# ChampiB/CBO_with_OOP

Measured on AMD Instinct MI355X. Metric: candidate-intervention acquisitions/sec (16k grid, d=3), higher is better.
Workload: dtype f64

## Files before the change

### cbo_with_oop_amd/csrc/cbo_api.hip

```cpp
#include <algorithm>
#include <atomic>
#include <cmath>
#include <cstdio>
#include <cstdlib>
#include <chrono>
#include <cstring>
#include <mutex>
#include <string>
#include <map>
#include <utility>
#include <vector>

#include "cbo_internal.h"
#include "hyper_prior.h"
#include "lml_outputs.h"
#include "schedule_tuner.h"

using namespace cbo;

static thread_local std::string g_err;
static std::atomic<uint64_t> g_fit_stamp{0};

static int fail(int code, const std::string &msg)
{
// ... 347 lines not shown
                if (c->bulk_stream) { hipStreamDestroy(c->bulk_stream); c->bulk_stream = nullptr; }
            }
        }
        if (!masked) {
            e = hipStreamCreateWithPriority(&c->sweep_stream, hipStreamNonBlocking, (prio_low + prio_high) / 2);
            if (e == hipSuccess) e = hipStreamCreateWithPriority(&c->bulk_stream, hipStreamNonBlocking, prio_low);
        }
    }
    if (e == hipSuccess) e = hipEventCreateWithFlags(&c->ev_join, hipEventDisableTiming | hipEventDisableSystemFence);
    if (e == hipSuccess) e = hipEventCreateWithFlags(&c->ev_join2, hipEventDisableTiming | hipEventDisableSystemFence);
    if (e == hipSuccess) e = hipEventCreateWithFlags(&c->ev_fork, hipEventDisableTiming | hipEventDisableSystemFence);
    if (e == hipSuccess) e = hipMalloc(&c->part_val, 2048 * sizeof(double));
    if (e == hipSuccess) e = hipMalloc(&c->part_idx, 2048 * sizeof(int64_t));
    if (e == hipSuccess) e = hipMalloc(&c->best_val, sizeof(double));
    if (e == hipSuccess) e = hipMalloc(&c->best_idx, sizeof(int64_t));
    if (e == hipSuccess) e = hipHostMalloc(&c->h_best_val, sizeof(double));
    if (e == hipSuccess) e = hipHostMalloc(&c->h_best_idx, sizeof(int64_t));
    if (e == hipSuccess) e = hipHostMalloc(&c->h_info, sizeof(int));
    if (e == hipSuccess) e = hipHostMalloc(&c->stage, kStageBytes);
    if (e == hipSuccess) e = hipEventCreateWithFlags(&c->stage_done, hipEventDisableTiming);
    if (e != hipSuccess) {
        destroy_ctx(c);
        return fail(CBO_ERR_HIP, std::string("cbo_init: ") + hipGetErrorString(e));
    }
    const char *ws = std::getenv("CBO_HIP_WORKSPACE_MB");
    if (ws) c->max_ws_bytes = (size_t)std::atoll(ws) << 20;
    c->n_cu = prop.multiProcessorCount;
    const char *sm = std::getenv("CBO_HIP_SWEEP");
    if (sm) c->sweep_mode = std::atoi(sm);
    const char *lr = std::getenv("CBO_HIP_LOO_ROUTE");
    if (lr) c->loo_route = std::atoi(lr);
    const char *hs = std::getenv("CBO_HIP_HYPER_SCHEDULE");
    if (hs) c->hyper_schedule = std::atoi(hs);
    const char *sc = std::getenv("CBO_HIP_SWEEP_CACHE");
    if (sc && std::atoi(sc) == 0) c->sweep_cache = false;
    const char *ss = std::getenv("CBO_HIP_SMALL_SETS");
    if (ss && std::atoi(ss) == 0) c->small_sets = false;
    const char *om = std::getenv("CBO_HIP_OVERLAP");
    if (om) c->overlap_mode = std::atoi(om);
    const char *tf = std::getenv("CBO_HIP_PIPE_TAIL");
    if (tf) c->pipe_tail_frac = std::atof(tf);
    const char *pg = std::getenv("CBO_HIP_PIPE_GROUP");
    if (pg) c->pipe_group = std::min(std::max(std::atoi(pg), 0), 4);
    const char *pl = std::getenv("CBO_HIP_PIPE_LEAD");
    if (pl) c->pipe_lead = std::atoi(pl);
    const char *pf = std::getenv("CBO_HIP_PANEL_FORM");
    if (pf && (std::atoi(pf) == 2 || std::atoi(pf) == 5)) c->chol.panel_form = std::atoi(pf);
    const char *sl = std::getenv("CBO_HIP_FUSED_SPIN_LIMIT");
    if (sl) c->chol.spin_limit = std::atoi(sl);
    const char *bg = std::getenv("CBO_HIP_BULK_GROUP");
    if (bg) c->chol.bulk_group = std::atoi(bg);
    const char *g4 = std::getenv("CBO_HIP_BULK_GROUP4_ROWS");
    if (g4) c->chol.group4_rows = std::atoi(g4);
    const char *vf = std::getenv("CBO_HIP_VEC_SOLVE_FORM");
    if (vf) c->vec_solve_form = std::atoi(vf);
    {
        static std::once_flag once;
        std::call_once(once, [] { std::atexit(shutdown_all_at_exit); });
        std::lock_guard<std::mutex> lock(g_live_mutex);
        g_live.push_back(c);
    }
    *out = c;
    return CBO_OK;
}

namespace cbo {
hipStream_t ctx_stream(cbo_ctx *c) { return c->stream; }
int ctx_device(cbo_ctx *c) { return c->device; }
}

extern "C" void cbo_shutdown(cbo_ctx *c)
{
    if (!c) return;
    {
        std::lock_guard<std::mutex> lock(g_live_mutex);
        auto it = std::find(g_live.begin(), g_live.end(), c);
        if (it == g_live.end()) return;
        g_live.erase(it);
    }
    destroy_ctx(c);
}

static void destroy_ctx(cbo_ctx *c)
{
    hipSetDevice(c->device);
    if (c->scratch_k) { cbo_cands_destroy(c->scratch_k); c->scratch_k = nullptr; }
    if (c->stream) hipStreamSynchronize(c->stream);
    for (auto &p : c->pending) { hipEventDestroy(p.a); hipEventDestroy(p.b); }
    for (auto e : c->pool) hipEventDestroy(e);
    hipFree(c->part_val); hipFree(c->part_idx); hipFree(c->best_val); hipFree(c->best_idx);
    hipHostFree(c->h_best_val); hipHostFree(c->h_best_idx); hipHostFree(c->h_info); hipHostFree(c->stage);
    if (c->stage_done) hipEventDestroy(c->stage_done);
    for (auto e : c->chol_events) hipEventDestroy(e);
    for (auto e : c->pipe_events) hipEventDestroy(e);
    if (c->region_a) hipEventDestroy(c->region_a);
    if (c->region_b) hipEventDestroy(c->region_b);
    if (c->ev_join) hipEventDestroy(c->ev_join);
    if (c->ev_join2) hipEventDestroy(c->ev_join2);
    if (c->ev_fork) hipEventDestroy(c->ev_fork);
    if (c->sweep_stream) hipStreamDestroy(c->sweep_stream);
    if (c->bulk_stream) hipStreamDestroy(c->bulk_stream);
    if (c->side_stream) hipStreamDestroy(c->side_stream);
    if (c->stream) hipStreamDestroy(c->stream);
    delete c;
}

// ... 665 lines not shown
    const int64_t max_cols = (int64_t)(c->max_ws_bytes / (elem * (size_t)n_pad)) / kStrip * kStrip;
    if (cols > max_cols) cols = max_cols < kStrip ? kStrip : max_cols;
    const int64_t ld = cols + (int64_t)(128 / elem);
    int rc = grow(c, c->V, (elem * (size_t)n_pad * (size_t)ld + sizeof(double) - 1) / sizeof(double));
    if (rc == CBO_OK) rc = grow_vectors(c, m_pad);
    if (rc != CBO_OK) return rc;
    *chunk_cols = cols;
    *ldv = ld;
    return CBO_OK;
}

static int prepare_cands(cbo_gp *g, cbo_cands *k)
{
    cbo_ctx *c = g->ctx;
    if (k->prepared_for == g && k->prepared_ls == g->ls) return CBO_OK;
    launch_prep_points(c->stream, k->raw, k->m, k->d, g->h.ard ? g->ls_dev : nullptr, k->has_prior ? k->pv : nullptr,
                       k->P.xs, k->m_pad, k->P.sq, k->has_prior ? k->P.sv : nullptr);
    HIP_TRY(hipGetLastError());
    k->prepared_for = g;
    k->prepared_ls = g->ls;
    return CBO_OK;
}

static void pipe_mark(void *user, hipStream_t st, int begin, double flops)
{
    cbo_ctx *c = static_cast<cbo_ctx *>(user);
    if (!c->profiling) return;
    EventPair &cur = c->pipe_cur;
    if (begin) {
        cur.a = get_event(c);
        cur.b = get_event(c);
        cur.phase = PH_TRSM;
        hipEventRecord(cur.a, st);
        c->timers.n_trsm_launches += 1;
        c->timers.trsm_flops += flops;
    } else {
        hipEventRecord(cur.b, st);
        c->pending.push_back(cur);
    }
}

static SweepPipe make_pipe(cbo_gp *g, double *V, int64_t ldv, int64_t cols, double *q, double *mu)
{
    cbo_ctx *c = g->ctx;
    SweepPipe pipe{};
    pipe.stream = c->sweep_stream;
    pipe.bulk = c->bulk_stream;
    pipe.V = V; pipe.ldv = ldv; pipe.m_pad = cols;
    pipe.zvec = g->z; pipe.q = q; pipe.mu = mu;
    pipe.events = &c->pipe_events;
    pipe.mark = pipe_mark; pipe.user = c;
    pipe.tail_begin = (int)g->n_pad;
    pipe.group = 0;
    return pipe;
}

static bool prefer_right_looking(const cbo_ctx *c, int64_t n_pad, int64_t cols)
{
    if (c->sweep_mode == 0) return false;
    if (c->sweep_mode == 1) return true;
    if (n_pad < 1024) return false;
    const int64_t strips = cols / kStrip;
    const int64_t rounds = (strips + c->n_cu - 1) / c->n_cu;
    return rounds * c->n_cu * 5 >= strips * 6;
}


static int enqueue_right_looking(cbo_gp *g, double *V, int64_t ldv, int64_t cols, double *q, double *mu,
                                 bool lower_tri = false)
{
    cbo_ctx *c = g->ctx;
    SweepPipe pipe = make_pipe(g, V, ldv, cols, q, mu);
    pipe.lower_tri = lower_tri;
    HIP_TRY(hipMemsetAsync(q, 0, sizeof(double) * cols, c->stream));
    HIP_TRY(hipMemsetAsync(mu, 0, sizeof(double) * cols, c->stream));
    int p = 0;
    for (int r0 = 0; r0 < (int)g->n_pad; r0 += 256, ++p)
        sweep_pipe_pair(pipe, c->stream, g->A, g->lda, g->invDt, g->n_pad, p, r0,
                        (r0 + 256 <= (int)g->n_pad) ? 256 : 128);
    HIP_TRY(hipEventRecord(c->ev_join, c->sweep_stream));
    HIP_TRY(hipStreamWaitEvent(c->stream, c->ev_join, 0));
    HIP_TRY(hipEventRecord(c->ev_join2, c->bulk_stream));
    HIP_TRY(hipStreamWaitEvent(c->stream, c->ev_join2, 0));
    return CBO_OK;
}

static int own_solution_buffer(cbo_gp *g, cbo_cands *k, double **V, int64_t *ldv)
{
    cbo_ctx *c = g->ctx;
    if (!k->V || k->v_rows_cap != g->n_pad || k->v_ld != k->m_pad + kLdExtra) {
        HIP_TRY(hipStreamSynchronize(c->stream));
        hipFree(k->V); hipFree(k->partial);
        k->V = nullptr; k->partial = nullptr; k->v_stamp = 0;
        k->v_ld = k->m_pad + kLdExtra;
        HIP_TRY(hipMalloc(&k->V, sizeof(double) * (size_t)g->n_pad * (size_t)k->v_ld));
        HIP_TRY(hipMalloc(&k->partial, sizeof(double) * 64 * (size_t)k->m_pad));
        k->v_rows_cap = g->n_pad;
    }
    *V = k->V;
    *ldv = k->v_ld;
    return CBO_OK;
}

static int enqueue_posterior_f32(cbo_gp *g, cbo_cands *k)
{
    cbo_ctx *c = g->ctx;
// ... 3042 lines not shown
    for (int j = 0, q = 0; j < ns + nm; ++j) {
        const cbo_mle_run &r = runs[taken[(size_t)j]];
        const size_t P = (size_t)r.n_params;
        for (int s = 0; s < r.n_starts; ++s, ++q) {
            if (c->mle_status[q] == kNoStatus) return fail(CBO_ERR_HIP, "MLE kernel: no status for a run it was given");
            r.status_out[s] = c->mle_status[q];
            r.rounds_out[s] = c->mle_rounds[q];
            if (r.status_out[s] == CBO_MLE_NOT_PD) continue;
            const double *fin = c->mle_final.p + (size_t)q * kFinal;
            std::memcpy(r.theta_out + (size_t)s * P, fin, sizeof(double) * P);
            r.lml_out[s] = fin[CBO_HMC_MAX_PARAMS];
            std::memcpy(r.grad_out + (size_t)s * P, fin + CBO_HMC_MAX_PARAMS + 1, sizeof(double) * P);
        }
    }
    return CBO_OK;
}

extern "C" int cbo_gp_mle_sets(int n_models, cbo_gp *const *gps, const cbo_mle_run *runs, int *model_status_out)
{
    return cbo_gp_mle_sets_rows(n_models, gps, runs, kPadN, model_status_out);
}

static int general_lml_gradients(cbo_gp *g, double *lml_out, double *dvariance_out, double *dlengthscale_out,
                                 double *dnoise_out)
{
    cbo_ctx *c = g->ctx;
    if (!g->fitted) {
        if (g->n_pad != kPadN) return fail(CBO_ERR_NOT_FITTED, "gp is not fitted");
        const int frc = cbo_gp_fit(g, nullptr, nullptr);
        if (frc != CBO_OK) return frc;
    }
    int rc = ensure_alpha(g);
    if (rc != CBO_OK) return rc;
    const int64_t n_pad = g->n_pad;
    int64_t chunk = 0, ldv = 0;
    rc = ensure_workspaces(c, n_pad, n_pad, &chunk, &ldv);
    if (rc != CBO_OK) return rc;
    if (chunk < n_pad) return fail(CBO_ERR_UNSUPPORTED, "likelihood gradients need an n_pad x n_pad workspace (raise CBO_HIP_WORKSPACE_MB)");
    const int64_t ldw = n_pad + kLdExtra;
    const size_t w_bytes = sizeof(double) * (size_t)n_pad * (size_t)ldw;
    rc = grow(c, c->W, (size_t)n_pad * (size_t)ldw);
    if (rc == CBO_OK) rc = grow(c, c->gpart, (size_t)lml_grad_tiles(n_pad) * (size_t)(1 + g->d));
    if (rc != CBO_OK) return rc;
    launch_set_identity(c->stream, c->V, ldv, n_pad);
    if (prefer_right_looking(c, n_pad, n_pad)) {
        rc = enqueue_right_looking(g, c->V, ldv, n_pad, c->q, c->mu, true);
        if (rc != CBO_OK) return rc;
    } else {
        launch_trsm_strips(c->stream, g->A, g->lda, g->invDt, c->V, ldv, n_pad, n_pad, g->z, c->q, c->mu);
    }
    HIP_TRY(hipMemsetAsync(c->W, 0, w_bytes, c->stream));
    for (int k0 = 0; k0 < (int)n_pad; k0 += 256) {
        const int klen = (k0 + 256 <= (int)n_pad) ? 256 : 128;
        launch_gemm_update(c->stream, c->V, ldv, c->V, ldv, c->W, ldw, k0, klen, 0, k0 + klen, k0 + klen, true);
    }
    launch_lml_grad(c->stream, g->X, g->h, g->alpha, c->W, ldw, n_pad, c->gpart, c->part_val);
    launch_lml_terms(c->stream, g->A, g->lda, n_pad, g->z, c->part_val + 16);
    HIP_TRY(hipGetLastError());
    launch_dot2(c->stream, g->alpha, g->alpha, g->n, c->part_val + 20);
    launch_sum(c->stream, c->q, g->n, c->part_val + 22);
    HIP_TRY(hipGetLastError());
    double hs[24];
    HIP_TRY(hipMemcpyAsync(hs, c->part_val, sizeof(hs), hipMemcpyDeviceToHost, c->stream));
    HIP_TRY(hipStreamSynchronize(c->stream));
    lml_outputs(g, hs, hs[16], hs[17], hs[20], hs[22], lml_out, dvariance_out, dlengthscale_out, dnoise_out);
    return CBO_OK;
}

static int general_loo(cbo_gp *g, double *mean_out, double *var_out, double *lpd_out, double *sum_out)
{
    cbo_ctx *c = g->ctx;
    int rc = ensure_alpha(g);
    if (rc != CBO_OK) return rc;
    const int64_t n_pad = g->n_pad;
    int64_t chunk = 0, ldv = 0;
    rc = ensure_workspaces(c, n_pad, n_pad, &chunk, &ldv);
    if (rc != CBO_OK) return rc;
    const int nb = loo_finish_blocks(g->n);
    rc = grow(c, c->gpart, (size_t)nb + 1);
    if (rc != CBO_OK) return rc;
    if (c->loo_route != 1 && c->loo_route != 2 && chunk >= n_pad && prefer_right_looking(c, n_pad, n_pad)) {
        launch_set_identity(c->stream, c->V, ldv, n_pad);
        rc = enqueue_right_looking(g, c->V, ldv, n_pad, c->q, c->mu, true);
        if (rc != CBO_OK) return rc;
    } else {
        for (int64_t c0 = 0; c0 < n_pad; c0 += chunk) {
            const int64_t cols = (n_pad - c0 < chunk) ? (n_pad - c0) : chunk;
            const int64_t r0 = c->loo_route == 2 ? 0 : c0 / 256 * 256;
            const int64_t rows = n_pad - r0;
            PhaseScope ps(c, PH_TRSM);
            launch_loo_identity_chunk(c->stream, c->V, ldv, rows, cols, c0 - r0);
            launch_trsm_strips(c->stream, g->A + r0 * g->lda + r0, g->lda, g->invDt + (r0 / 16) * 256, c->V, ldv, rows,
                               cols, g->z + r0, c->q + c0, c->mu + c0);
            if (c->profiling) {
                c->timers.n_trsm_launches += 1;
                c->timers.trsm_flops += (double)rows * (double)rows * (double)cols;
            }
        }
    }
    double *partial = c->gpart, *sum_dev = c->gpart + nb;
    launch_loo_finish(c->stream, c->q, g->alpha, g->y, g->n, mean_out ? c->mean.p : nullptr, var_out ? c->var.p : nullptr,
                      lpd_out ? c->acq.p : nullptr, partial, sum_dev);
    HIP_TRY(hipGetLastError());
    const size_t bytes = sizeof(double) * (size_t)g->n;
    if (mean_out) HIP_TRY(hipMemcpyAsync(mean_out, c->mean, bytes, hipMemcpyDeviceToHost, c->stream));
    if (var_out) HIP_TRY(hipMemcpyAsync(var_out, c->var, bytes, hipMemcpyDeviceToHost, c->stream));
    if (lpd_out) HIP_TRY(hipMemcpyAsync(lpd_out, c->acq, bytes, hipMemcpyDeviceToHost, c->stream));
// ... 452 lines not shown
```

### cbo_with_oop_amd/csrc/cbo_internal.h

```cpp
#pragma once

#include <hip/hip_runtime.h>
#include <cstddef>
#include <cstdint>
#include <string>
#include <vector>

#include "cbo_hip.h"

namespace cbo {

typedef double d4 __attribute__((ext_vector_type(4)));
typedef double d2 __attribute__((ext_vector_type(2)));

#if defined(__HIP_DEVICE_COMPILE__) || defined(__HIPCC__)
typedef __attribute__((address_space(3))) void *lds_ptr_t;
__device__ __forceinline__ void glds16(const double *gsrc, unsigned lds_dst)
{
    unsigned keep;
    asm volatile("s_mov_b32 %0, m0\n\ts_mov_b32 m0, %2\n\ts_nop 0\n\tglobal_load_lds_dwordx4 %1, off\n\ts_mov_b32 m0, %0"
                 : "=&s"(keep)
                 : "v"(gsrc), "s"(lds_dst)
                 : "memory");
}
// ... 58 lines not shown
    int n_k;
    const double *xs1, *sq1, *sv1, *xs2, *sq2, *sv2; int64_t ldx;
    int64_t m1, m2;
    double *C; int64_t ldc;
    double variance, inv_l2, noise;
    int zero_diag, tiles;
};
void launch_cov_tiles(hipStream_t s, int d, bool sym, CovArgs a);
struct SampArgs {
    const double *U; int64_t ldu;
    const double *Z; int64_t ldz;
    const double *mean;
    int64_t m, s;
    double *F; int64_t ldf;
    int tiles_i, tiles_j;
};
void launch_samples_tiles(hipStream_t st, SampArgs a);
void launch_normals_transpose(hipStream_t st, const double *normals, int64_t m, int64_t s, double *Z, int64_t m_pad,
                              int64_t ldz);
void launch_factor_padding(hipStream_t st, double *A, int64_t lda, int64_t m, int64_t m_pad);
constexpr int kJointTile = 128;
struct IvrArgs {
    const double *Vc, *Vi; int64_t ldv, c_cols, i_cols;
    int n_k;
    const double *xs1, *sq1, *sv1, *xs2, *sq2, *sv2; int64_t ldx;
    int64_t m, p;
    double *part; int64_t ldp; int64_t tile0;
    double variance, inv_l2;
};
void launch_ivr_tiles(hipStream_t s, int d, IvrArgs a);
void launch_ivr_finish(hipStream_t s, const double *part, int64_t ldp, int tiles, const double *var, int64_t m, double p,
                       double cost, double *ivr, double *part_val, int64_t *part_idx, int n_blocks);
int ivr_finish_blocks_for(int64_t m);
constexpr int kPadN32 = 256;
void launch_factor_to_f32(hipStream_t s, const double *A, int64_t lda, int64_t n_pad, const double *invDt, float *Uf,
                          int64_t ldu, float *invF, int64_t n32);
void launch_kstar_f32(hipStream_t s, const PointSet &X, const PointSet &C, int64_t c_begin, int64_t m_pad,
                      const KernelHyper &h, float *V, int64_t ldv, int64_t n32, const double *alpha, double *mu_part,
                      double *mu);
void launch_trsm_strips_f32(hipStream_t s, const float *U, int64_t ldu, const float *invDt, float *V, int64_t ldv,
                            int64_t n32, int64_t m_pad, double *q);
int run_mfma_f32_selftest(hipStream_t s, double *max_err);

struct SweepPipe {
    hipStream_t stream;
    hipStream_t bulk;
    double *V;
    int64_t ldv, m_pad;
    double *zvec;
    double *q, *mu;
    bool lower_tri;
    int group;
    int lead = 0;
    int tail_begin;
    std::vector<hipEvent_t> *events;
    void (*mark)(void *user, hipStream_t st, int begin, double flops);
    void *user;
};
constexpr int kCholFlagSlots = 1024;
constexpr int kCholFusedTimeout = -2147483647 - 1;
constexpr int kFusedSpinLimit = 1 << 22;
struct CholOptions {
    int panel_form = 4;
    int spin_limit = kFusedSpinLimit;
    int bulk_group = 4;
    int group4_rows = 10240;
};
void launch_cholesky(hipStream_t s, hipStream_t side, std::vector<hipEvent_t> &events, double *A, int64_t lda,
                     int64_t n_pad, double *invDt, int *info_dev, const CholOptions &opt, const SweepPipe *pipe = nullptr,
                     bool info_zeroed = false);
inline int cholesky_info_ints(int64_t n_pad)
{
    const int np = (int)(n_pad / 128);
    return 2 * np <= kCholFlagSlots ? 1 + 2 * np : 1;
}
void sweep_pipe_pair(const SweepPipe &pipe, hipStream_t chain, const double *A, int64_t lda, const double *invDt,
                     int64_t n_pad, int p, int r0, int klen);
void sweep_pipe_tail(const SweepPipe &pipe, hipStream_t chain, const double *A, int64_t lda, const double *invDt,
                     int64_t n_pad, int pairs_done);
void launch_backsolve(hipStream_t s, const double *A, int64_t lda, int64_t n_pad, const double *invDt, double *alpha);
void launch_forward_vec(hipStream_t s, const double *A, int64_t lda, int64_t n_pad, const double *invDt, double *w,
                        double *out);
void launch_gather_column(hipStream_t s, const double *V, int64_t ldv, int64_t n_pad, double *dst);
bool launch_backsolve_chain(hipStream_t s, const double *A, int64_t lda, int64_t n_pad, const double *invDt,
                            const double *src, int64_t src_stride, double *work, double *out, int *info, int spin_limit,
                            int form);
bool launch_forward_chain(hipStream_t s, const double *A, int64_t lda, int64_t n_pad, const double *invDt, const double *w,
                          double *out, int *info, int spin_limit, int form);
void launch_backsolve_vec(hipStream_t s, const double *A, int64_t lda, int64_t n_pad, const double *invDt,
                          const double *src, int64_t src_stride, double *work, double *out);
void launch_pred_gradients(hipStream_t s, const PointSet &X, int64_t n_pad, const PointSet &C, int64_t c_begin,
                           int64_t cols, int64_t m, const KernelHyper &h, const double *inv_ls_dev, const double *alpha,
                           const double *W, int64_t ldw, double *dmean, double *dvar);
void launch_reversed_factor(hipStream_t s, const double *A, int64_t lda, int64_t n_pad, const double *invDt, double *T,
                            int64_t ldt, double *invT);
void launch_reverse_rows(hipStream_t s, const double *V, int64_t ldv, int64_t n_pad, int64_t cols, double *W, int64_t ldw);
void launch_dot2(hipStream_t s, const double *a, const double *b, int64_t n, double *out2);
void launch_sum(hipStream_t s, const double *a, int64_t n, double *out);
void launch_expand_interventions(hipStream_t s, const double *observed, int64_t n_obs, int d, const double *values, int n_iv,
                                 const int *iv_index, int64_t m, double *raw);

void launch_trsm_strips(hipStream_t s, const double *U, int64_t ldu, const double *invDt, double *V, int64_t ldv,
                        int64_t n, int64_t m_pad, const double *z, double *q, double *mu, bool accumulate = false,
                        bool half_lds = false);
void launch_gemm_update(hipStream_t s, const double *U, int64_t ldu, const double *V, int64_t ldv, double *C,
                        int64_t ldc, int k0, int klen, int i0_begin, int i0_end, int64_t m_pad, bool upper_only,
                        const int *skip_if = nullptr);

struct cbo_small_set {
    const double *xs, *sq, *sv, *pm, *y;
    const double *cxs, *csq, *csv, *cpm, *cpv;
    int64_t ld, cld, m, index_offset;
    int n, d, zero_diag, task;
    double variance, lengthscale, noise_var, diag_add, y_best, ei_jitter, cost;
    int ard, pad_;
    const double *stage, *stage_ls;
    double *raw, *pv;
};
struct cbo_small_result {
    double best_val;
    int64_t best_idx;
    int info;
    int seq;
};
size_t small_sets_scratch_doubles(int n_sets, int blocks_per_set);
constexpr int kSmallLmlTerms = 1 + CBO_MAX_DIM + 4;
struct cbo_small_lml_result {
    double terms[kSmallLmlTerms];
    int info, seq;
};
size_t small_lml_scratch_doubles();
void launch_small_lml(hipStream_t s, const cbo_small_set &st, double *scratch, int *info, cbo_small_lml_result *out, int seq);
size_t mid_lml_scratch_doubles();
void launch_small_lml_batch(hipStream_t s, const cbo_small_set *sets, int n_models, double *scratch, int64_t stride,
                            int *info, cbo_small_lml_result *out, int seq);
struct cbo_small_loo_result {
    double sum;
    double mean[128], var[128], lpd[128];
    int info, seq;
};
size_t small_loo_scratch_doubles();
void launch_small_loo_batch(hipStream_t s, const cbo_small_set *sets, int n_models, double *scratch, int *info,
                            cbo_small_loo_result *out, int seq);
void launch_loo_identity_chunk(hipStream_t s, double *V, int64_t ldv, int64_t rows, int64_t cols, int64_t shift);
int loo_finish_blocks(int64_t n);
void launch_loo_finish(hipStream_t s, const double *c, const double *alpha, const double *y, int64_t n, double *mean_out,
                       double *var_out, double *lpd_out, double *partial, double *sum_out);
constexpr int kSmallTwoPhaseFromBlocks = 12;
constexpr int kEiKind = 0;
constexpr int kMesKind = 5;
constexpr int kPredictKind = 6;
constexpr int kLogEiKind = 7;
constexpr int kEiPointKind = 8;
constexpr int kLogEiPointKind = 9;
struct cbo_small_aux {
    int64_t off, count;
};
struct SmallAux {
    const cbo_small_aux *per_set = nullptr;
    const double *data = nullptr;
// ... 283 lines not shown
```

### cbo_with_oop_amd/csrc/kernels_chol.hip

```cpp
#include <hip/hip_ext.h>
#include <climits>
#include <atomic>
#include <cstring>
#include <vector>

#include "cbo_mid_lml_device.h"

namespace cbo {

__global__ __launch_bounds__(256) void potrf_diag128_v2_kernel(double *A, int64_t lda, int r0, int rcol,
                                                               double *__restrict__ invDt, int *info,
                                                               double *__restrict__ zvec)
{
    extern __shared__ __align__(16) unsigned char smem_raw[];
    Diag2Shared &sh = *reinterpret_cast<Diag2Shared *>(smem_raw);
    if (__builtin_nontemporal_load(info) != 0) return;
    const int tid = threadIdx.x;
    const int lane = tid & 63;
    const int wave = __builtin_amdgcn_readfirstlane(tid >> 6);
    {
        const unsigned s0 = lds_byte_address(&sh.S[0][0]);
        const double *g = A + (int64_t)(r0 + wave * 32) * lda + r0 + lane * 2;
#pragma unroll 8
        for (int p = 0; p < 32; ++p) {
// ... 469 lines not shown
static void launch_syrk_rows(hipStream_t s, double *A, int64_t lda, int r0, int n1, int n2, int rcol, const int *skip_if,
                             int rows = 128, hipEvent_t done = nullptr)
{
    const int c0 = r0 + n1;
    const int nt = n2 / 64;
    if (nt <= 0) { if (done) hipEventRecord(done, s); return; }
    if (rows > n2) rows = n2;
    hipExtLaunchKernelGGL(syrk_rows_kernel, dim3(nt + 1, rows / 32), dim3(256), 0, s, nullptr, done, 0, A, lda, r0, n1, c0,
                          nt, rcol, skip_if);
}

static void launch_syrk(hipStream_t s, double *A, int64_t lda, int r0, int n1, int n2, int rcol, int ti_begin,
                        int ti_end, const int *skip_if)
{
    const int c0 = r0 + n1;
    const int nt = n2 / 64;
    if (ti_end > nt) ti_end = nt;
    if (ti_end <= ti_begin) return;
    hipLaunchKernelGGL(syrk_kernel<64>, dim3(nt + 1, ti_end - ti_begin), dim3(256), 0, s, A, lda, r0, n1, c0, nt, rcol,
                       ti_begin, skip_if);
}

static hipEvent_t event_slot(std::vector<hipEvent_t> &ev, size_t i)
{
    while (ev.size() <= i) {
        hipEvent_t e;
        hipEventCreateWithFlags(&e, hipEventDisableTiming | hipEventDisableSystemFence);
        ev.push_back(e);
    }
    return ev[i];
}

void sweep_pipe_pair(const SweepPipe &pipe, hipStream_t chain, const double *A, int64_t lda, const double *invDt,
                     int64_t n_pad, int p, int r0, int klen)
{
    auto pipe_event = [&](int kind, int pp) {
        return event_slot(*pipe.events, (size_t)(3 * pp + kind));
    };
    const int64_t cols = (pipe.lower_tri && r0 + klen < pipe.m_pad) ? (int64_t)(r0 + klen) : pipe.m_pad;
    const double m = (double)cols;
    hipEventRecord(pipe_event(0, p), chain);
    hipStreamWaitEvent(pipe.stream, pipe_event(0, p), 0);
    if (pipe.mark) pipe.mark(pipe.user, pipe.stream, 1, (double)klen * (double)klen * m);
    launch_trsm_strips(pipe.stream, A + (int64_t)r0 * lda + r0, lda, invDt + (int64_t)(r0 / 16) * 256,
                       pipe.V + (int64_t)r0 * pipe.ldv, pipe.ldv, klen, cols, pipe.zvec + r0, pipe.q, pipe.mu, true, true);
    if (pipe.mark) pipe.mark(pipe.user, pipe.stream, 0, 0.0);
    hipEventRecord(pipe_event(1, p), pipe.stream);
    const int below = r0 + klen;
    if (below >= (int)n_pad) return;
    const int first_end = (below + 256 < (int)n_pad) ? below + 256 : (int)n_pad;
    auto update = [&](hipStream_t st, int k0, int kl, int i0, int i1) {
        if (i0 >= i1) return;
        if (pipe.mark) pipe.mark(pipe.user, st, 1, 2.0 * (double)kl * (double)(i1 - i0) * m);
        launch_gemm_update(st, A, lda, pipe.V, pipe.ldv, pipe.V, pipe.ldv, k0, kl, i0, i1, cols, false);
        if (pipe.mark) pipe.mark(pipe.user, st, 0, 0.0);
    };
    const int G = pipe.group, lead = pipe.lead;
    const int full_pairs = ((pipe.tail_begin < (int)n_pad) ? pipe.tail_begin : (int)n_pad) / 256;
    const bool grouped = G >= 2 && !pipe.lower_tri && klen == 256 && p >= lead && ((p - lead) / G + 1) * G + lead <= full_pairs;
    if (grouped) {
        const int j = (p - lead) / G, i = (p - lead) % G;
        const int g0 = 256 * (lead + G * j);
        const int next_end = (g0 + 512 * G < (int)n_pad) ? g0 + 512 * G : (int)n_pad;
        if (i == 0 && j == 0 && lead > 0) hipStreamWaitEvent(pipe.stream, pipe_event(2, lead - 1), 0);
        update(pipe.stream, r0, 256, below, first_end);
        if (i == 0 && j >= 1) hipStreamWaitEvent(pipe.stream, pipe_event(2, lead + G * (j - 1)), 0);
        update(pipe.stream, r0, 256, r0 + 512, next_end);
        if (i < G - 1) return;
        hipStreamWaitEvent(pipe.bulk, pipe_event(1, p), 0);
        const int a1 = (g0 + 768 * G < (int)n_pad) ? g0 + 768 * G : (int)n_pad;
        update(pipe.bulk, g0, 256 * G, next_end, a1);
        hipEventRecord(pipe_event(2, lead + G * j), pipe.bulk);
        update(pipe.bulk, g0, 256 * G, a1, (int)n_pad);
        hipEventRecord(pipe_event(2, p), pipe.bulk);
        return;
    }
    if (p > 0) hipStreamWaitEvent(pipe.stream, pipe_event(2, p - 1), 0);
    update(pipe.stream, r0, klen, below, first_end);
    hipStreamWaitEvent(pipe.bulk, pipe_event(1, p), 0);
    update(pipe.bulk, r0, klen, first_end, (int)n_pad);
    hipEventRecord(pipe_event(2, p), pipe.bulk);
}

void sweep_pipe_tail(const SweepPipe &pipe, hipStream_t chain, const double *A, int64_t lda, const double *invDt,
                     int64_t n_pad, int pairs_done)
{
    std::vector<hipEvent_t> &ev = *pipe.events;
    const hipEvent_t last = event_slot(ev, (size_t)(3 * pairs_done));
    if (pairs_done > 0) {
        hipEventRecord(last, pipe.stream);
        hipStreamWaitEvent(chain, last, 0);
        hipStreamWaitEvent(chain, ev[(size_t)(3 * (pairs_done - 1) + 2)], 0);
    }
    const int t0 = pipe.tail_begin;
    const double rows = (double)((int)n_pad - t0);
    if (pipe.mark) pipe.mark(pipe.user, chain, 1, rows * rows * (double)pipe.m_pad);
    launch_trsm_strips(chain, A + (int64_t)t0 * lda + t0, lda, invDt + (int64_t)(t0 / 16) * 256,
                       pipe.V + (int64_t)t0 * pipe.ldv, pipe.ldv, (int64_t)n_pad - t0, pipe.m_pad, pipe.zvec + t0, pipe.q,
                       pipe.mu, true, false);
    if (pipe.mark) pipe.mark(pipe.user, chain, 0, 0.0);
}

__global__ void zero_ints_kernel(int *p, int n)
{
    for (int i = threadIdx.x; i < n; i += blockDim.x) p[i] = 0;
}

void launch_cholesky(hipStream_t s, hipStream_t side, std::vector<hipEvent_t> &events, double *A, int64_t lda,
                     int64_t n_pad, double *invDt, int *info_dev, const CholOptions &opt, const SweepPipe *pipe,
                     bool info_zeroed)
{
    hipFuncSetAttribute(reinterpret_cast<const void *>(potrf_diag128_v2_kernel), hipFuncAttributeMaxDynamicSharedMemorySize,
                        (int)sizeof(Diag2Shared));
    hipFuncSetAttribute(reinterpret_cast<const void *>(panel_trsm_kernel), hipFuncAttributeMaxDynamicSharedMemorySize,
                        (int)sizeof(PanelShared));
    hipFuncSetAttribute(reinterpret_cast<const void *>(potrf_panel_fused_kernel), hipFuncAttributeMaxDynamicSharedMemorySize,
                        (int)sizeof(Diag2Shared));
    constexpr int syrk_gemm_rows = 6144;
    auto launch_diag = [&](int rr) {
        hipLaunchKernelGGL(potrf_diag128_v2_kernel, dim3(1), dim3(256), sizeof(Diag2Shared), s, A, lda, rr, (int)n_pad,
                           invDt, info_dev, pipe ? pipe->zvec : nullptr);
    };
    const int np = (int)(n_pad / 128);
    const bool fused = opt.panel_form != 2 && 2 * np <= kCholFlagSlots;
    const bool split = opt.panel_form == 5;
    if (!info_zeroed) hipLaunchKernelGGL(zero_ints_kernel, dim3(1), dim3(256), 0, s, info_dev, fused ? 1 + 2 * np : 1);
    int *flags = info_dev + 1;
    const int rcol = (int)n_pad;
    event_slot(events, (size_t)(2 * np + 1));
    hipEventRecord(events[2 * np], s);
    hipStreamWaitEvent(side, events[2 * np], 0);
    double *zvec = pipe ? pipe->zvec : nullptr;
    const bool lean_panel = !pipe;
    int pair = 0;
    auto sweep_rows = [&](int r0, int klen) {
        if (pipe && r0 < pipe->tail_begin) sweep_pipe_pair(*pipe, s, A, lda, invDt, n_pad, pair++, r0, klen);
    };
    int pending = -1;
    int group_left = 0;
    int group_pairs = 0, group_g0 = 0, group_first_k = 0;
    int pending_big_a = -1;
    for (int k = 0; k < np; k += 2) {
        const int r0 = 128 * k;
        const int n2 = (int)n_pad - r0 - 128;
        const int n3_pair = (int)n_pad - r0 - 256;
        if (group_left == 0 && opt.bulk_group >= 2 && (fused || lean_panel)) {
            int G = 0;
            if (opt.bulk_group >= 4 && n3_pair - 1024 >= opt.group4_rows && n3_pair - 1024 >= syrk_gemm_rows &&
                n3_pair - 1024 >= 1024)
                G = 4;
            else if (n3_pair - 512 >= syrk_gemm_rows && n3_pair - 512 >= 512) G = 2;
            if (G != 0) { group_pairs = G; group_left = G; group_g0 = r0; group_first_k = k; }
        }
        const bool grouped = group_left > 0;
        const bool first_of_group = grouped && group_left == group_pairs;
        const bool last_of_group = grouped && group_left == 1;
        const bool split_now = split || grouped;
        auto factor_panel = [&](int r, int cols, hipEvent_t done) {
            if (fused && cols > 0) {
                launch_panel_fused(s, A, lda, r, rcol, invDt, info_dev, zvec, cols, flags + 2 * (r / 128), opt.spin_limit,
                                   done, split_now);
                return;
            }
            launch_diag(r);
            if (cols <= 0) return;
            if (lean_panel) launch_panel_trsm(s, A, lda, r, r + 128, cols, invDt, info_dev, done);
            else
                launch_trsm_strips(s, A + (int64_t)r * lda + r, lda, invDt + (int64_t)(r / 16) * 256,
                                   A + (int64_t)r * lda + r + 128, lda, 128, cols, nullptr, nullptr, nullptr, false, true);
        };
        factor_panel(r0, n2, nullptr);
        if (n2 <= 0) { sweep_rows(r0, 128); break; }
        launch_syrk_rows(s, A, lda, r0, 128, n2, rcol, info_dev);
        const int r1 = r0 + 128;
        const int n3 = (int)n_pad - r1 - 128;
        const bool bulk = n3 > 256;
        const bool gemm_form = bulk && n3 - 256 >= syrk_gemm_rows;
        const bool carried = bulk && (fused || lean_panel);
        const hipEvent_t ev_panel = (carried && gemm_form && (!grouped || last_of_group)) ? events[2 * k] : nullptr;
        const hipEvent_t ev_rows = (carried && !gemm_form) ? events[2 * k] : nullptr;
        factor_panel(r1, n3, ev_panel);
        sweep_rows(r0, 256);
        if (n3 <= 0) break;
        if (grouped) {
            const int S = 256 * group_pairs, g0 = group_g0, n = (int)n_pad;
            const int next_end = (g0 + 2 * S < n) ? g0 + 2 * S : n;
            if (last_of_group) {
                hipStreamWaitEvent(side, events[2 * k], 0);
                const int a_end = (g0 + 3 * S < n) ? g0 + 3 * S : n;
                launch_gemm_update(side, A, lda, A, lda, A, lda, g0, S, next_end, a_end, n_pad + kRhsCols, true, info_dev);
                hipEventRecord(events[2 * group_first_k + 1], side);
                pending_big_a = 2 * group_first_k + 1;
                if (a_end < n)
                    launch_gemm_update(side, A, lda, A, lda, A, lda, g0, S, a_end, n, n_pad + kRhsCols, true, info_dev);
                hipEventRecord(events[2 * k + 1], side);
                pending = 2 * k + 1;
            }
            launch_syrk_rows(s, A, lda, r0, 256, n3, rcol, info_dev, 256, nullptr);
            if (first_of_group && pending_big_a >= 0) hipStreamWaitEvent(s, events[pending_big_a], 0);
            launch_gemm_update(s, A, lda, A, lda, A, lda, r0, 256, r0 + 512, next_end, n_pad + kRhsCols, true, info_dev);
            --group_left;
            continue;
        }
        const int prev = pending;
        auto launch_bulk = [&] {
            if (!carried) hipEventRecord(events[2 * k], s);
            hipStreamWaitEvent(side, events[2 * k], 0);
            if (gemm_form)
                launch_gemm_update(side, A, lda, A, lda, A, lda, r0, 256, r0 + 256 + 256, (int)n_pad, n_pad + kRhsCols, true,
                                   info_dev);
            else
                launch_syrk(side, A, lda, r0, 256, n3, rcol, 4, n3 / 64, info_dev);
            hipEventRecord(events[2 * k + 1], side);
            pending = 2 * k + 1;
        };
        if (gemm_form) launch_bulk();
        if (prev >= 0) hipStreamWaitEvent(s, events[prev], 0);
        launch_syrk_rows(s, A, lda, r0, 256, n3, rcol, info_dev, 256, ev_rows);
        if (bulk && !gemm_form) launch_bulk();
    }
    hipEventRecord(events[2 * np + 1], side);
    hipStreamWaitEvent(s, events[2 * np + 1], 0);
    if (pipe && pipe->tail_begin < (int)n_pad) sweep_pipe_tail(*pipe, s, A, lda, invDt, n_pad, pair);
}

__global__ __launch_bounds__(256) void backsolve_step_kernel(const double *__restrict__ A, int64_t lda,
                                                             const double *__restrict__ invDt, int blk, double *zt,
                                                             double *__restrict__ alpha)
{
    __shared__ double zs[128];
    __shared__ double al[128];
    const int tid = threadIdx.x;
    const int lane = tid & 63, wave = tid >> 6;
    const int b0 = blk * 128;
    if (tid < 128) zs[tid] = zt[b0 + tid];
    __syncthreads();
    for (int s = 7; s >= 0; --s) {
        const int o = 16 * s;
        if (tid < 64) {
            const int i = tid >> 2, part = tid & 3;
            const double *Y = invDt + (int64_t)(b0 / 16 + s) * 256;
            double acc = 0.0;
#pragma unroll
            for (int k = 0; k < 4; ++k) acc = fma(Y[i * 16 + 4 * part + k], zs[o + 4 * part + k], acc);
            acc += __shfl_xor(acc, 1);
            acc += __shfl_xor(acc, 2);
            if (part == 0) al[o + i] = acc;
        }
        __syncthreads();
        if (tid < o) {
            const double *row = A + (int64_t)(b0 + tid) * lda + b0 + o;
            double acc = zs[tid];
#pragma unroll
            for (int c = 0; c < 16; ++c) acc = fma(-row[c], al[o + c], acc);
            zs[tid] = acc;
        }
        __syncthreads();
    }
    const int g = blockIdx.x;
    if (g == blk) {
        if (tid < 128) alpha[b0 + tid] = al[tid];
        return;
    }
// ... 292 lines not shown
```

### cbo_with_oop_amd/csrc/kernels_trsm.hip

```cpp
#include <cstdlib>
#include <type_traits>

#include "cbo_internal.h"

namespace cbo {

#define MFMA_F64(a, b, c) __builtin_amdgcn_mfma_f64_16x16x4f64((a), (b), (c), 0, 0, 0)

#define SCHED_DS(n) __builtin_amdgcn_sched_group_barrier(0x100, (n), 0)
#define SCHED_MFMA(n) __builtin_amdgcn_sched_group_barrier(0x008, (n), 0)
#define SCHED_VMEM(n) __builtin_amdgcn_sched_group_barrier(0x010, (n), 0)

constexpr int kRB = 128;
constexpr int kT = kRB / 16;
constexpr int kLdsLd = kRB + 16;
constexpr int kNBuf = 3;
template <int KB>
struct StageGeom {
    static constexpr int kA = KB * kLdsLd;
    static constexpr int kB = 4 * KB * 16;
    static constexpr int kRA = KB / 4;
    static constexpr int kParts = KB / 8;
    static constexpr int kDma = 3 * kParts;
    static constexpr int kKS = KB / 4;
    static constexpr int kDiagStages = kRB / KB;
    static constexpr int kDiagTiles = KB / 16;
    static constexpr int kDiagStores = 4 * kDiagTiles;
    static_assert(kParts <= kKS - 2, "the DMA groups and the cursor update ride under the first k-steps");
};

struct StageCursor {
    int i0, j, lim;
    int ai0, aj;
    const double *a_src;
    const double *b_src;
    int64_t b_stride;
};

template <bool SWEEP, int KB>
__global__ __launch_bounds__(256) void trsm_strip_kernel(const double *__restrict__ U, int64_t ldu,
                                                         const double *__restrict__ invDt, double *V, int64_t ldv,
                                                         int n, const double *__restrict__ z,
                                                         double *__restrict__ q_out, double *__restrict__ mu_out,
                                                         int accumulate)
{
    using G = StageGeom<KB>;
    constexpr int kKB = KB, kABuf = G::kA, kBBuf = G::kB, kDmaPerStage = G::kDma, kStoresPerDiagStage = G::kDiagStores;
    constexpr int kDS = G::kDiagStages, kDT = G::kDiagTiles, kKS = G::kKS, kParts = G::kParts;
    __shared__ __align__(16) double lds[kNBuf * (kABuf + kBBuf)];

    const int tid = threadIdx.x;
    const int lane = tid & 63;
    const int wave = __builtin_amdgcn_readfirstlane(tid >> 6);
    const int lc = lane & 15, kq = lane >> 4;
    const int64_t colw = (int64_t)blockIdx.x * kStrip + wave * 16;
    double *Vc = V + colw + lc;
    double *ldsB = lds + kNBuf * kABuf;
    const unsigned lds_byte0 = lds_byte_address(lds);
    const double *ug = U + (int64_t)(wave * G::kRA) * ldu + lane * 2;
    const double *vg = V + (int64_t)(lane >> 3) * ldv + colw + 2 * (lane & 7);

    const double *inv_lane = invDt + lane * 2;
    auto locate_a = [&](StageCursor &c) __attribute__((always_inline)) {
        const bool past = c.i0 >= n;
        c.ai0 = past ? n - kRB : c.i0;
        c.aj = past ? (n - kRB) / kKB + kDS - 1 : c.j;
    };
    auto locate_b = [&](StageCursor &c) __attribute__((always_inline)) {
        c.a_src = ug + (int64_t)(kKB * c.aj) * ldu + c.ai0;
    };
    auto locate_c = [&](StageCursor &c) __attribute__((always_inline)) {
        const int nreg = c.ai0 / kKB;
        const int64_t diag = (c.aj >= nreg) ? 1 : 0;
        const int64_t off_diag = ((int64_t)(c.ai0 / 16) + kDT * (c.aj - nreg)) * 256;
        const int64_t off_reg = (int64_t)(kKB * c.aj) * ldv;
        const uintptr_t base = (uintptr_t)vg + ((uintptr_t)inv_lane - (uintptr_t)vg) * (uintptr_t)diag;
        c.b_src = reinterpret_cast<const double *>(base) + (off_reg + (off_diag - off_reg) * diag);
        c.b_stride = 8 * ldv + (128 - 8 * ldv) * diag;
    };
    auto locate = [&](StageCursor &c) __attribute__((always_inline)) {
        locate_a(c);
        locate_b(c);
        locate_c(c);
    };
    auto step = [&](StageCursor &c) __attribute__((always_inline)) {
        const int wrap = (c.j + 1 == c.lim) ? 1 : 0;
        c.i0 += kRB * wrap;
        c.j = (c.j + 1) * (1 - wrap);
        c.lim = c.lim + (c.i0 / kKB + kDS - c.lim) * wrap;
    };
    auto advance = [&](StageCursor &c) __attribute__((always_inline)) {
        step(c);
        locate(c);
// ... 1025 lines not shown
                    for (int t = s + 2; t < kT; ++t)
#pragma unroll
                        for (int kk = 0; kk < 4; ++kk) uf[1][t][kk] = ab[(4 * kk) * kPLd + kRB + 16 * t];
                    const d4 y = y1 + y2;
                    emit(1, y);
#pragma unroll
                    for (int kk = 0; kk < 4; ++kk)
#pragma unroll
                        for (int t = s + 2; t < kT; ++t) {
                            acc[t] = MFMA_F64(uf[1][t][kk], y[kk], acc[t]);
                            const int idx = kk * (kT - s - 2) + (t - s - 2);
                            if (m < 2 && idx < 16) request_one(i0, 16 * m + idx);
                        }
                    a1 += 8 + (m == 0 ? kL0 : m == 1 ? kL1 : 0);
                    if (SWEEP && m == kPD1 - 1) {
                        qacc += __shfl_xor(qacc, 16);
                        qacc += __shfl_xor(qacc, 32);
                        macc += __shfl_xor(macc, 16);
                        macc += __shfl_xor(macc, 32);
                        qtot += qacc;
                        mtot += macc;
                        qacc = 0.0;
                        macc = 0.0;
                    }
                    buf = (buf == 2) ? 0 : buf + 1;
                }
            }
        };
        diag_phase(0, std::true_type{});
        for (int i0 = kPB; i0 < n; i0 += kPB) {
            const int nst = i0 / kPKB;
            regular_stage(i0, std::true_type{});
            for (int j = 1; j < nst; ++j) regular_stage(i0, std::false_type{});
            diag_phase(i0, std::false_type{});
        }
        asm volatile("s_waitcnt vmcnt(0)" ::: "memory");
        __builtin_amdgcn_s_barrier();

        if (SWEEP && H == 1 && kq == 0) {
            q_out[colw + lc] = qtot;
            mu_out[colw + lc] = mtot;
        }
    };
    if (h == 0) run(std::integral_constant<int, 0>{});
    else run(std::integral_constant<int, 1>{});
}

constexpr int kAccMoves = kT * 4;

template <int KB>
__global__ __launch_bounds__(256) void trsm_update_kernel(const double *__restrict__ U, int64_t ldu,
                                                          const double *V, int64_t ldv, double *C, int64_t ldc, int k0,
                                                          int klen, int i0_begin, int i0_end, int chunk_rows,
                                                          int upper_only, const int *__restrict__ skip_if)
{
    if (skip_if && __builtin_nontemporal_load(skip_if) != 0) return;
    using G = StageGeom<KB>;
    constexpr int kA = G::kA, kB = G::kB, kRA = G::kRA, kParts = G::kParts, kDma = G::kDma, kKS = G::kKS;
    __shared__ __align__(16) double lds[kNBuf * (kA + kB)];

    const int tid = threadIdx.x;
    const int lane = tid & 63;
    const int wave = __builtin_amdgcn_readfirstlane(tid >> 6);
    const int lc = lane & 15, kq = lane >> 4;
    const int64_t colw = (int64_t)blockIdx.x * kStrip + wave * 16;
    const int ib = i0_begin + (int)blockIdx.y * chunk_rows;
    const int ie = (ib + chunk_rows < i0_end) ? ib + chunk_rows : i0_end;
    if (ib >= ie) return;
    if (upper_only && (int)blockIdx.x * kStrip + kStrip <= ib) return;
    const int nst = klen / KB;
    double *Cc = C + colw + lc;
    double *ldsB = lds + kNBuf * kA;
    const unsigned lds_byte0 = lds_byte_address(lds);
    const double *ug = U + (int64_t)(k0 + wave * kRA) * ldu + lane * 2;
    const double *vg = V + (int64_t)(k0 + (lane >> 3)) * ldv + colw + 2 * (lane & 7);
    const int64_t b_stride = 8 * ldv;

    int ci0 = ib, cj = 0;
    const double *a_src, *b_src;
    auto locate = [&]() __attribute__((always_inline)) {
        const bool past = ci0 >= ie;
        const int ai0 = past ? ie - kRB : ci0;
        const int aj = past ? nst - 1 : cj;
        a_src = ug + (int64_t)(KB * aj) * ldu + ai0;
        b_src = vg + (int64_t)(KB * aj) * ldv;
    };
    auto advance = [&]() __attribute__((always_inline)) {
        const int wrap = (cj + 1 == nst) ? 1 : 0;
        ci0 += kRB * wrap;
        cj = (cj + 1) * (1 - wrap);
        locate();
    };
    auto issue_one = [&](int buf, int part, int q) __attribute__((always_inline)) {
        if (q < 2) {
            const unsigned la = __builtin_amdgcn_readfirstlane(lds_byte0 + 8u * (unsigned)(buf * kA + (wave * kRA) * kLdsLd));
            const int p = 2 * part + q;
            glds16(a_src + (int64_t)p * ldu, la + 8u * (unsigned)(p * kLdsLd));
        } else {
            const unsigned lb = __builtin_amdgcn_readfirstlane(
                lds_byte0 + 8u * (unsigned)(kNBuf * kA + buf * kB + wave * (KB * 16)));
            glds16(b_src + part * b_stride, lb + 8u * (unsigned)(part * 128));
        }
    };
    auto issue_part = [&](int buf, int part) __attribute__((always_inline)) {
#pragma unroll
        for (int q = 0; q < 3; ++q) issue_one(buf, part, q);
    };

    d4 acc[kT], accn[kT];
#pragma unroll
    for (int t = 0; t < kT; ++t)
#pragma unroll
        for (int r = 0; r < 4; ++r) acc[t][r] = -Cc[(int64_t)(ib + 16 * t + kq + 4 * r) * ldc];

    locate();
#pragma unroll
    for (int part = 0; part < kParts; ++part) issue_part(0, part);
    advance();
#pragma unroll
    for (int part = 0; part < kParts; ++part) issue_part(1, part);
    advance();

// ... 50 lines not shown
                }
            }
            deferred = true;
            buf = (buf == 2) ? 0 : buf + 1;
        }
#pragma unroll
        for (int t = 0; t < kT; ++t) acc[t] = MFMA_F64(af[1][t], bf[1], acc[t]);
#pragma unroll
        for (int t = 0; t < kT; ++t)
#pragma unroll
            for (int r = 0; r < 4; ++r) Cc[(int64_t)(i0 + 16 * t + kq + 4 * r) * ldc] = -acc[t][r];
        asm volatile("" ::: "memory");
#pragma unroll
        for (int t = 0; t < kT; ++t) acc[t] = accn[t];
        boundary = 2;
    }
    asm volatile("s_waitcnt vmcnt(0)" ::: "memory");
    __builtin_amdgcn_s_barrier();
}

void launch_trsm_strips(hipStream_t s, const double *U, int64_t ldu, const double *invDt, double *V, int64_t ldv,
                        int64_t n, int64_t m_pad, const double *z, double *q, double *mu, bool accumulate,
                        bool half_lds)
{
    if (n <= 0 || m_pad <= 0) return;
    const dim3 grid((unsigned)(m_pad / kStrip));
    const int acc = accumulate ? 1 : 0;
    if (half_lds) {
        if (q != nullptr)
            hipLaunchKernelGGL((trsm_strip_kernel<true, 16>), grid, dim3(256), 0, s, U, ldu, invDt, V, ldv, (int)n, z, q, mu, acc);
        else
            hipLaunchKernelGGL((trsm_strip_kernel<false, 16>), grid, dim3(256), 0, s, U, ldu, invDt, V, ldv, (int)n, z, q, mu, 0);
        return;
    }
    static const bool pairs = [] {
        const char *e = getenv("CBO_HIP_STRIP_FORM");
        return !(e && atoi(e) == 8);
    }();
    if (pairs && n >= kPB && n % kPB == 0) {
        if (q != nullptr)
            hipLaunchKernelGGL((trsm_pair_kernel<true>), grid, dim3(512), 0, s, U, ldu, invDt, V, ldv, (int)n, z, q, mu, acc);
        else
            hipLaunchKernelGGL((trsm_pair_kernel<false>), grid, dim3(512), 0, s, U, ldu, invDt, V, ldv, (int)n, z, q, mu, 0);
        return;
    }
    if (q != nullptr)
        hipLaunchKernelGGL((trsm_strip8_kernel<true>), grid, dim3(512), 0, s, U, ldu, invDt, V, ldv, (int)n, z, q, mu, acc);
    else
        hipLaunchKernelGGL((trsm_strip8_kernel<false>), grid, dim3(512), 0, s, U, ldu, invDt, V, ldv, (int)n, z, q, mu, 0);
}

void launch_gemm_update(hipStream_t s, const double *U, int64_t ldu, const double *V, int64_t ldv, double *C,
                        int64_t ldc, int k0, int klen, int i0_begin, int i0_end, int64_t m_pad, bool upper_only,
                        const int *skip_if)
{
    if (i0_begin >= i0_end || m_pad <= 0 || klen <= 0) return;
    const dim3 grid((unsigned)(m_pad / kStrip), (unsigned)((i0_end - i0_begin + kRB - 1) / kRB));
    const int up = upper_only ? 1 : 0;
    hipLaunchKernelGGL(trsm_update_kernel<16>, grid, dim3(256), 0, s, U, ldu, V, ldv, C, ldc, k0, klen, i0_begin, i0_end, kRB,
                       up, skip_if);
}

__global__ void mfma_selftest_kernel(const double *A, const double *B, double *C)
{
    const int l = threadIdx.x;
    d4 acc = {0.0, 0.0, 0.0, 0.0};
    for (int k0 = 0; k0 < 16; k0 += 4)
        acc = MFMA_F64(A[(l & 15) * 16 + k0 + (l >> 4)], B[(k0 + (l >> 4)) * 16 + (l & 15)], acc);
    d4 acc2 = {0.0, 0.0, 0.0, 0.0};
    for (int kk = 0; kk < 4; ++kk) acc2 = MFMA_F64(A[(l & 15) * 16 + 4 * kk + (l >> 4)], acc[kk], acc2);
    for (int r = 0; r < 4; ++r) {
        C[((l >> 4) + 4 * r) * 16 + (l & 15)] = acc[r];
        C[256 + ((l >> 4) + 4 * r) * 16 + (l & 15)] = acc2[r];
    }
}

int run_mfma_selftest(hipStream_t s, double *max_err)
{
    double hA[256], hB[256], hC[512], ref[256], ref2[256];
    for (int i = 0; i < 16; ++i)
        for (int j = 0; j < 16; ++j) {
            hA[i * 16 + j] = (double)((i * 7 + j * 3) % 11 - 5);
            hB[i * 16 + j] = (double)((i * 5 + j * 13 + 1) % 17 - 8);
        }
    for (int i = 0; i < 16; ++i)
        for (int j = 0; j < 16; ++j) {
            double acc = 0.0;
            for (int k = 0; k < 16; ++k) acc += hA[i * 16 + k] * hB[k * 16 + j];
            ref[i * 16 + j] = acc;
        }
    for (int i = 0; i < 16; ++i)
        for (int j = 0; j < 16; ++j) {
            double acc = 0.0;
            for (int k = 0; k < 16; ++k) acc += hA[i * 16 + k] * ref[k * 16 + j];
            ref2[i * 16 + j] = acc;
        }
    double *dA = nullptr, *dB = nullptr, *dC = nullptr;
    if (hipMalloc(&dA, sizeof(hA)) != hipSuccess || hipMalloc(&dB, sizeof(hB)) != hipSuccess ||
        hipMalloc(&dC, sizeof(hC)) != hipSuccess)
        return -1;
    hipMemcpyAsync(dA, hA, sizeof(hA), hipMemcpyHostToDevice, s);
    hipMemcpyAsync(dB, hB, sizeof(hB), hipMemcpyHostToDevice, s);
    hipLaunchKernelGGL(mfma_selftest_kernel, dim3(1), dim3(64), 0, s, dA, dB, dC);
    hipMemcpyAsync(hC, dC, sizeof(hC), hipMemcpyDeviceToHost, s);
    const hipError_t e = hipStreamSynchronize(s);
    hipFree(dA); hipFree(dB); hipFree(dC);
    if (e != hipSuccess) return -1;
    double m = 0.0;
    for (int i = 0; i < 256; ++i) {
        const double e1 = fabs(hC[i] - ref[i]), e2 = fabs(hC[256 + i] - ref2[i]);
        if (e1 > m) m = e1;
        if (e2 > m) m = e2;
    }
// ... 6 lines not shown
```

Before: 3.082 million.

## Add XCD-aware grouped tile ordering for GEMM update kernel

Adds an optional remapping of workgroup IDs in the trailing GEMM update kernel. Tiles are grouped by strip ranges assigned to each of eight round-robin dispatch labels (matching the MI355X XCDs) and walked in column groups, so that workgroups sharing an XCD's L2 reuse the same operand panels. The option is controlled by a new env knob that defaults to 0, which keeps the original linear order. It also adds an occupancy hint of 2 blocks per SIMD to the KB=16 strip TRSM kernel, which may force register spills.

After: 3.094 million, median of 6. Within noise of the previous version (+0.4%).

```diff
diff --git a/cbo_with_oop_amd/csrc/cbo_api.hip b/cbo_with_oop_amd/csrc/cbo_api.hip
--- a/cbo_with_oop_amd/csrc/cbo_api.hip
+++ b/cbo_with_oop_amd/csrc/cbo_api.hip
@@ -423,6 +423,8 @@
     if (bg) c->chol.bulk_group = std::atoi(bg);
     const char *g4 = std::getenv("CBO_HIP_BULK_GROUP4_ROWS");
     if (g4) c->chol.group4_rows = std::atoi(g4);
+    const char *tg = std::getenv("CBO_HIP_UPDATE_TILE_GROUP");
+    if (tg) c->chol.update_tile_group = std::min(std::max(std::atoi(tg), 0), 64);
     const char *vf = std::getenv("CBO_HIP_VEC_SOLVE_FORM");
     if (vf) c->vec_solve_form = std::atoi(vf);
     {
@@ -1194,6 +1196,7 @@
     pipe.mark = pipe_mark; pipe.user = c;
     pipe.tail_begin = (int)g->n_pad;
     pipe.group = 0;
+    pipe.tile_group = c->chol.update_tile_group;
     return pipe;
 }
 
@@ -4342,7 +4345,7 @@
     HIP_TRY(hipMemsetAsync(c->W, 0, w_bytes, c->stream));
     for (int k0 = 0; k0 < (int)n_pad; k0 += 256) {
         const int klen = (k0 + 256 <= (int)n_pad) ? 256 : 128;
-        launch_gemm_update(c->stream, c->V, ldv, c->V, ldv, c->W, ldw, k0, klen, 0, k0 + klen, k0 + klen, true);
+        launch_gemm_update(c->stream, c->V, ldv, c->V, ldv, c->W, ldw, k0, klen, 0, k0 + klen, k0 + klen, true, c->chol.update_tile_group);
     }
     launch_lml_grad(c->stream, g->X, g->h, g->alpha, c->W, ldw, n_pad, c->gpart, c->part_val);
     launch_lml_terms(c->stream, g->A, g->lda, n_pad, g->z, c->part_val + 16);
diff --git a/cbo_with_oop_amd/csrc/cbo_internal.h b/cbo_with_oop_amd/csrc/cbo_internal.h
--- a/cbo_with_oop_amd/csrc/cbo_internal.h
+++ b/cbo_with_oop_amd/csrc/cbo_internal.h
@@ -134,6 +134,7 @@
     bool lower_tri;
     int group;
     int lead = 0;
+    int tile_group = 0;
     int tail_begin;
     std::vector<hipEvent_t> *events;
     void (*mark)(void *user, hipStream_t st, int begin, double flops);
@@ -147,6 +148,7 @@
     int spin_limit = kFusedSpinLimit;
     int bulk_group = 4;
     int group4_rows = 10240;
+    int update_tile_group = 0;
 };
 void launch_cholesky(hipStream_t s, hipStream_t side, std::vector<hipEvent_t> &events, double *A, int64_t lda,
                      int64_t n_pad, double *invDt, int *info_dev, const CholOptions &opt, const SweepPipe *pipe = nullptr,
@@ -187,7 +189,7 @@
                         bool half_lds = false);
 void launch_gemm_update(hipStream_t s, const double *U, int64_t ldu, const double *V, int64_t ldv, double *C,
                         int64_t ldc, int k0, int klen, int i0_begin, int i0_end, int64_t m_pad, bool upper_only,
-                        const int *skip_if = nullptr);
+                        int tile_group, const int *skip_if = nullptr);
 
 struct cbo_small_set {
     const double *xs, *sq, *sv, *pm, *y;
diff --git a/cbo_with_oop_amd/csrc/kernels_chol.hip b/cbo_with_oop_amd/csrc/kernels_chol.hip
--- a/cbo_with_oop_amd/csrc/kernels_chol.hip
+++ b/cbo_with_oop_amd/csrc/kernels_chol.hip
@@ -545,7 +545,7 @@
     auto update = [&](hipStream_t st, int k0, int kl, int i0, int i1) {
         if (i0 >= i1) return;
         if (pipe.mark) pipe.mark(pipe.user, st, 1, 2.0 * (double)kl * (double)(i1 - i0) * m);
-        launch_gemm_update(st, A, lda, pipe.V, pipe.ldv, pipe.V, pipe.ldv, k0, kl, i0, i1, cols, false);
+        launch_gemm_update(st, A, lda, pipe.V, pipe.ldv, pipe.V, pipe.ldv, k0, kl, i0, i1, cols, false, pipe.tile_group);
         if (pipe.mark) pipe.mark(pipe.user, st, 0, 0.0);
     };
     const int G = pipe.group, lead = pipe.lead;
@@ -610,6 +610,7 @@
     hipFuncSetAttribute(reinterpret_cast<const void *>(potrf_panel_fused_kernel), hipFuncAttributeMaxDynamicSharedMemorySize,
                         (int)sizeof(Diag2Shared));
     constexpr int syrk_gemm_rows = 6144;
+    const int tile_group = opt.update_tile_group;
     auto launch_diag = [&](int rr) {
         hipLaunchKernelGGL(potrf_diag128_v2_kernel, dim3(1), dim3(256), sizeof(Diag2Shared), s, A, lda, rr, (int)n_pad,
                            invDt, info_dev, pipe ? pipe->zvec : nullptr);
@@ -681,17 +682,17 @@
             if (last_of_group) {
                 hipStreamWaitEvent(side, events[2 * k], 0);
                 const int a_end = (g0 + 3 * S < n) ? g0 + 3 * S : n;
-                launch_gemm_update(side, A, lda, A, lda, A, lda, g0, S, next_end, a_end, n_pad + kRhsCols, true, info_dev);
+                launch_gemm_update(side, A, lda, A, lda, A, lda, g0, S, next_end, a_end, n_pad + kRhsCols, true, tile_group, info_dev);
                 hipEventRecord(events[2 * group_first_k + 1], side);
                 pending_big_a = 2 * group_first_k + 1;
                 if (a_end < n)
-                    launch_gemm_update(side, A, lda, A, lda, A, lda, g0, S, a_end, n, n_pad + kRhsCols, true, info_dev);
+                    launch_gemm_update(side, A, lda, A, lda, A, lda, g0, S, a_end, n, n_pad + kRhsCols, true, tile_group, info_dev);
                 hipEventRecord(events[2 * k + 1], side);
                 pending = 2 * k + 1;
             }
             launch_syrk_rows(s, A, lda, r0, 256, n3, rcol, info_dev, 256, nullptr);
             if (first_of_group && pending_big_a >= 0) hipStreamWaitEvent(s, events[pending_big_a], 0);
-            launch_gemm_update(s, A, lda, A, lda, A, lda, r0, 256, r0 + 512, next_end, n_pad + kRhsCols, true, info_dev);
+            launch_gemm_update(s, A, lda, A, lda, A, lda, r0, 256, r0 + 512, next_end, n_pad + kRhsCols, true, tile_group, info_dev);
             --group_left;
             continue;
         }
@@ -701,7 +702,7 @@
             hipStreamWaitEvent(side, events[2 * k], 0);
             if (gemm_form)
                 launch_gemm_update(side, A, lda, A, lda, A, lda, r0, 256, r0 + 256 + 256, (int)n_pad, n_pad + kRhsCols, true,
-                                   info_dev);
+                                   tile_group, info_dev);
             else
                 launch_syrk(side, A, lda, r0, 256, n3, rcol, 4, n3 / 64, info_dev);
             hipEventRecord(events[2 * k + 1], side);
diff --git a/cbo_with_oop_amd/csrc/kernels_trsm.hip b/cbo_with_oop_amd/csrc/kernels_trsm.hip
--- a/cbo_with_oop_amd/csrc/kernels_trsm.hip
+++ b/cbo_with_oop_amd/csrc/kernels_trsm.hip
@@ -2,6 +2,7 @@
 #include <type_traits>
 
 #include "cbo_internal.h"
+#include "tile_order.h"
 
 namespace cbo {
 
@@ -38,7 +39,7 @@
 };
 
 template <bool SWEEP, int KB>
-__global__ __launch_bounds__(256) void trsm_strip_kernel(const double *__restrict__ U, int64_t ldu,
+__global__ __launch_bounds__(256, KB == 16 ? 2 : 1) void trsm_strip_kernel(const double *__restrict__ U, int64_t ldu,
                                                          const double *__restrict__ invDt, double *V, int64_t ldv,
                                                          int n, const double *__restrict__ z,
                                                          double *__restrict__ q_out, double *__restrict__ mu_out,
@@ -1170,7 +1171,7 @@
 __global__ __launch_bounds__(256) void trsm_update_kernel(const double *__restrict__ U, int64_t ldu,
                                                           const double *V, int64_t ldv, double *C, int64_t ldc, int k0,
                                                           int klen, int i0_begin, int i0_end, int chunk_rows,
-                                                          int upper_only, const int *__restrict__ skip_if)
+                                                          int upper_only, const int *__restrict__ skip_if, int tile_group)
 {
     if (skip_if && __builtin_nontemporal_load(skip_if) != 0) return;
     using G = StageGeom<KB>;
@@ -1181,11 +1182,12 @@
     const int lane = tid & 63;
     const int wave = __builtin_amdgcn_readfirstlane(tid >> 6);
     const int lc = lane & 15, kq = lane >> 4;
-    const int64_t colw = (int64_t)blockIdx.x * kStrip + wave * 16;
-    const int ib = i0_begin + (int)blockIdx.y * chunk_rows;
+    const TileCoord tile = tile_order_map((int)(blockIdx.y * gridDim.x + blockIdx.x), (int)gridDim.x, (int)gridDim.y, tile_group);
+    const int64_t colw = (int64_t)tile.strip * kStrip + wave * 16;
+    const int ib = i0_begin + tile.row_block * chunk_rows;
     const int ie = (ib + chunk_rows < i0_end) ? ib + chunk_rows : i0_end;
     if (ib >= ie) return;
-    if (upper_only && (int)blockIdx.x * kStrip + kStrip <= ib) return;
+    if (upper_only && tile.strip * kStrip + kStrip <= ib) return;
     const int nst = klen / KB;
     double *Cc = C + colw + lc;
     double *ldsB = lds + kNBuf * kA;
@@ -1342,13 +1344,13 @@
 
 void launch_gemm_update(hipStream_t s, const double *U, int64_t ldu, const double *V, int64_t ldv, double *C,
                         int64_t ldc, int k0, int klen, int i0_begin, int i0_end, int64_t m_pad, bool upper_only,
-                        const int *skip_if)
+                        int tile_group, const int *skip_if)
 {
     if (i0_begin >= i0_end || m_pad <= 0 || klen <= 0) return;
     const dim3 grid((unsigned)(m_pad / kStrip), (unsigned)((i0_end - i0_begin + kRB - 1) / kRB));
     const int up = upper_only ? 1 : 0;
     hipLaunchKernelGGL(trsm_update_kernel<16>, grid, dim3(256), 0, s, U, ldu, V, ldv, C, ldc, k0, klen, i0_begin, i0_end, kRB,
-                       up, skip_if);
+                       up, skip_if, tile_group);
 }
 
 __global__ void mfma_selftest_kernel(const double *A, const double *B, double *C)
diff --git a/cbo_with_oop_amd/csrc/tile_order.h b/cbo_with_oop_amd/csrc/tile_order.h
--- /dev/null
+++ b/cbo_with_oop_amd/csrc/tile_order.h
@@ -0,0 +1,53 @@
+#pragma once
+
+#if defined(__HIPCC__) || defined(__CUDACC__)
+#define CBO_TILE_ORDER_HD __host__ __device__
+#else
+#define CBO_TILE_ORDER_HD
+#endif
+
+namespace cbo {
+
+constexpr int kTileOrderLabels = 8;
+
+struct TileCoord {
+    int strip, row_block;
+};
+
+CBO_TILE_ORDER_HD inline TileCoord tile_order_local(int k, int s0, int strips_c, int row_blocks, int group)
+{
+    const int per_group = group * row_blocks;
+    const int g = k / per_group, rem = k - g * per_group;
+    const int left = strips_c - g * group;
+    const int w = left < group ? left : group;
+    const int rb = rem / w;
+    return TileCoord{s0 + g * group + (rem - rb * w), rb};
+}
+
+CBO_TILE_ORDER_HD inline TileCoord tile_order_map(int id, int strips, int row_blocks, int group)
+{
+    if (group <= 0) return TileCoord{id % strips, id / strips};
+    constexpr int L = kTileOrderLabels;
+    const int total = strips * row_blocks;
+    const int q = strips / L, r = strips % L;
+    const int c = id % L, j = id / L;
+    auto range_begin = [&](int l) { return l * q + (l < r ? l : r); };
+    auto range_size = [&](int l) { return q + (l < r ? 1 : 0); };
+    auto tiles = [&](int l) { return range_size(l) * row_blocks; };
+    auto workgroups = [&](int l) { return (total - l + L - 1) / L; };
+    if (j < tiles(c)) return tile_order_local(j, range_begin(c), range_size(c), row_blocks, group);
+    int s = j - tiles(c);
+    for (int l = 0; l < c; ++l) {
+        const int over = workgroups(l) - tiles(l);
+        if (over > 0) s += over;
+    }
+    for (int l = 0; l < L; ++l) {
+        const int spare = tiles(l) - workgroups(l);
+        if (spare <= 0) continue;
+        if (s < spare) return tile_order_local(workgroups(l) + s, range_begin(l), range_size(l), row_blocks, group);
+        s -= spare;
+    }
+    return TileCoord{id % strips, id / strips};
+}
+
+}
```
